# lammps/lammps-plugins

Measured on AMD Instinct MI355X. Metric: Matom-steps/sec, higher is better.
Workload: dtype f64; 1 GPU; REBO-MoS bulk: in.rebomos-bulk cell replicated 24x24x24; atoms=3981312, style=rebomos, parallelism=spatial-dd1, transport=none (one GPU), rccl_library_is_test_double=False, thermo_every=10, displacement_check=every step, deferred on-device flag, dangerous_builds=0, inner_skin=adaptive from 1.0, late_style_list_builds_rank0=0, row_prunings_late_rank0=0, rccl_ranks=1

## Files before the change

### include/mdpair_hip.h

```cpp
#ifndef MDPAIR_HIP_H
#define MDPAIR_HIP_H

#include <stddef.h>
#include <stdint.h>

#ifdef __cplusplus
extern "C" {
#endif

#define MDP_ABI_VERSION 3

enum {
  MDP_OK = 0,
  MDP_EINVAL = -1,
  MDP_EHIP = -2,
  MDP_ENOMEM = -3,
  MDP_EOVERFLOW = -4,
  MDP_ENOTIMPL = -5,
  MDP_ESTATE = -6
};

#define MDP_EFLAG_GLOBAL 1
#define MDP_EFLAG_ATOM 2
#define MDP_VFLAG_GLOBAL 1
// ... 86 lines not shown

int mdp_md_setup(mdp_ctx *ctx, const mdp_md_config *cfg, const double *x, const double *v, const int *type,
                 const int *tag, const double *mass, const int *map, const int *ghost_owner,
                 const double *ghost_shift, const int *ghost_type, const int *ghost_tag);
int mdp_md_build_neighbors(mdp_ctx *ctx);
int mdp_md_initial_integrate(mdp_ctx *ctx);
int mdp_md_final_integrate(mdp_ctx *ctx);
int mdp_md_final_initial_integrate(mdp_ctx *ctx);
int mdp_md_defer_final(mdp_ctx *ctx);
int mdp_md_compute(mdp_ctx *ctx, int eflag, int vflag);
int mdp_md_compute_begin(mdp_ctx *ctx, int eflag, int vflag);
int mdp_md_compute_end(mdp_ctx *ctx, int eflag, int vflag);
int mdp_md_pack_x(mdp_ctx *ctx, int n, const int *d_sendlist, const double *d_shift, double *d_buf);
int mdp_md_unpack_x(mdp_ctx *ctx, int first_ghost, int n, const double *d_buf);
int mdp_md_pack_scalar(mdp_ctx *ctx, int which, int n, const int *d_sendlist, double *d_buf);
int mdp_md_unpack_scalar(mdp_ctx *ctx, int which, int first_ghost, int n, const double *d_buf);
int mdp_md_pack_ghost_f(mdp_ctx *ctx, int first_ghost, int n, double *d_buf);
int mdp_md_unpack_add_f(mdp_ctx *ctx, int n, const int *d_sendlist, const double *d_buf);
int mdp_md_fold_self_ghost_f(mdp_ctx *ctx);
int mdp_md_aeam_density(mdp_ctx *ctx, int eflag);
int mdp_md_aeam_force_begin(mdp_ctx *ctx, int eflag, int vflag);
int mdp_md_aeam_force(mdp_ctx *ctx, int eflag, int vflag);
int mdp_md_aeam_state(mdp_ctx *ctx, int out[4]);
int mdp_md_thermo(mdp_ctx *ctx, double out[9]);
int mdp_md_download(mdp_ctx *ctx, double *x, double *v, double *f, double *eatom);
int mdp_md_upload_x(mdp_ctx *ctx, const double *x);
int mdp_md_download_x_all(mdp_ctx *ctx, double *x_all);
void *mdp_md_ptr(mdp_ctx *ctx, const char *name);
int mdp_md_neighbor_stats(mdp_ctx *ctx, long long out[8]);
int mdp_md_prune_stats(mdp_ctx *ctx, long long out[4]);
int mdp_md_list_state(mdp_ctx *ctx, double out[8]);
int mdp_rebomos_list_info(mdp_ctx *ctx, long long out[8]);
int mdp_rebomos_centre_paths(mdp_ctx *ctx, long long out[2], int reset);
int mdp_md_class_stats(mdp_ctx *ctx, long long out[32]);

typedef struct {
  double boxlo[3];
  double h[6];
  int procgrid[3];
  int rank;
  double cutghost;
  int self_remote;
  int nonperiodic[3];
} mdp_dd_config;

int mdp_dd_setup(mdp_ctx *ctx, const mdp_dd_config *cfg);
int mdp_dd_reneighbor(mdp_ctx *ctx);
int mdp_dd_migrate_begin(mdp_ctx *ctx, int *send_counts );
int mdp_dd_migrate_pack(mdp_ctx *ctx, double *d_buf);
int mdp_dd_migrate_end(mdp_ctx *ctx, int narrive, const double *d_buf);
int mdp_dd_borders_begin(mdp_ctx *ctx, int *send_counts );
int mdp_dd_borders_pack(mdp_ctx *ctx, double *d_buf);
int mdp_dd_borders_end(mdp_ctx *ctx, const int *recv_counts , const double *d_buf);
int mdp_dd_info(mdp_ctx *ctx, long long out[8], int *send_counts, int *recv_counts);
int mdp_dd_forward_pack(mdp_ctx *ctx, double *d_buf);
int mdp_dd_forward_unpack(mdp_ctx *ctx, const double *d_buf);
int mdp_dd_forward_scalar_pack(mdp_ctx *ctx, double *d_buf);
int mdp_dd_forward_scalar_unpack(mdp_ctx *ctx, const double *d_buf);
int mdp_dd_reverse_pack(mdp_ctx *ctx, double *d_buf);
int mdp_dd_reverse_unpack(mdp_ctx *ctx, const double *d_buf);
int mdp_dd_comm_unique_id(void *id128);
int mdp_dd_comm_library(char *buf, int cap);
int mdp_dd_comm_init(mdp_ctx *ctx, const void *id128);
int mdp_dd_comm_destroy(mdp_ctx *ctx);
int mdp_dd_comm_reneighbor(mdp_ctx *ctx);
int mdp_dd_comm_forward_begin(mdp_ctx *ctx);
// ... 175 lines not shown
```

### lammps-plugins_amd/csrc/md.hip

```cpp
#include "mdp_common.h"

#include <rocprim/rocprim.hpp>

#include <cmath>
#include <type_traits>

void mdp_rebomos_fill_dev(mdp_ctx *c, double skin);

namespace {

struct CutTables {
  double owned[MDP_AEAM_MAXT * MDP_AEAM_MAXT];
  double ghost[MDP_AEAM_MAXT * MDP_AEAM_MAXT];
  const double *g_owned;
  int ne;
  int min_type;
};

using Grid = MdpGrid;

__device__ __forceinline__ int cell_index(const Grid &g, const double4 &x, int &cx, int &cy, int &cz)
{
  cx = (int) ((x.x - g.lo[0]) * g.inv[0]);
  cy = (int) ((x.y - g.lo[1]) * g.inv[1]);
// ... 1613 lines not shown
  if (!strcmp(name, "fp")) return c->fp.p;
  if (!strcmp(name, "eatom")) return c->eatom.p;
  return nullptr;
}

int mdp_rebomos_list_info(mdp_ctx *c, long long out[8])
{
  if (!c || !out) return MDP_EINVAL;
  if (!c->rebo_packed) return mdp_fail(c, MDP_ESTATE, "rebomos lists not built yet");
  out[0] = c->lj_tiled ? 1 : 0;
  out[1] = c->ntile;
  out[2] = c->tile_cap;
  out[3] = c->tile_maxu;
  out[4] = c->lj_total;
  out[5] = c->nclus;
  out[6] = (c->lj_class_base[2] - c->lj_class_base[1]) + (c->lj_class_base[4] - c->lj_class_base[3]);
  out[7] = c->style_builds;
  return MDP_OK;
}

int mdp_rebomos_centre_paths(mdp_ctx *c, long long out[2], int reset)
{
  if (!c || !out) return MDP_EINVAL;
  out[0] = out[1] = 0;
  if (!c->centre_paths.p) return MDP_OK;
  unsigned long long h[2];
  MDP_TRY(mdp_read_one(c, c->centre_paths.p, sizeof h, h));
  out[0] = (long long) h[0];
  out[1] = (long long) h[1];
  if (reset) MDP_HIP(c, hipMemsetAsync(c->centre_paths.p, 0, sizeof h, c->stream));
  return MDP_OK;
}

int mdp_md_class_stats(mdp_ctx *c, long long out[32])
{
  if (!c || !out) return MDP_EINVAL;
  for (int k = 0; k < 32; k++) out[k] = 0;
  out[30] = c->tile_maxu;
  if (c->cfg.style == 2 || (c->have_aeam && !c->have_rebomos)) {
    out[0] = c->h_ang_count;
    out[1] = c->ntile;
    out[2] = c->aeam_split;
    return MDP_OK;
  }
  for (int k = 0; k < MDP_NCLASS; k++) out[k] = c->h_class_count[k];
  for (int k = 0; k < 4; k++) out[20 + k] = c->lj_class_base[k + 1] - c->lj_class_base[k];
  if (c->lj_tiled && !c->lj_ordered) out[20] = c->ntile;
  if (c->h_pinned) {
    const int *h = mdp_pin(c, kPinOvf) + 4 * c->ovf_par;
    for (int k = 0; k < 4; k++) out[25 + k] = h[k];
    out[24] = *mdp_pin(c, kPinGeneral);
  }
  out[29] = c->tile_small;
  return MDP_OK;
}

int mdp_md_neighbor_stats(mdp_ctx *c, long long out[8])
{
  if (!c || !out) return MDP_EINVAL;
  for (int k = 0; k < 8; k++) out[k] = 0;
  out[0] = c->nb_owned_total;
  out[1] = c->nb_total - c->nb_owned_total;
  out[2] = c->lj_total;
  out[3] = c->cand_total;
  out[4] = 0;
  for (int k = 0; k < MDP_NCLASS; k++) out[4] += c->h_class_count[k];
// ... 110 lines not shown
```

### lammps-plugins_amd/csrc/rebomos.hip

```cpp
#include "mdp_common.h"

#include <type_traits>

#define MDP_SINPI_COEFFS 3.14159265358979312e+00, -5.16771278004996937e+00, 2.55016403987734508e+00, -5.99264529320791883e-01, 8.21458866111281910e-02, -7.37043094571434784e-03, 4.66302805767612337e-04, -2.19153534478302037e-05
#define MDP_COSPI_COEFFS 1.00000000000000000e+00, -4.93480220054467900e+00, 4.05871212641676760e+00, -1.33526276885458928e+00, 2.35330630358893123e-01, -2.58068913900140508e-02, 1.92957430940392206e-03, -1.04638104924845650e-04, 4.30306958703294391e-06
__constant__ double mdp_sinpi_series[8] = {MDP_SINPI_COEFFS};
__constant__ double mdp_cospi_series[9] = {MDP_COSPI_COEFFS};

namespace {

#ifndef MDP_LJ_WAVES
#define MDP_LJ_WAVES 4
#endif
constexpr double kPi = 3.14159265358979323846;
constexpr double kTol = 1.0e-9;

__device__ __forceinline__ void wave_lds_fence()
{
  __builtin_amdgcn_fence(__ATOMIC_RELEASE, "wavefront");
  __builtin_amdgcn_wave_barrier();
  __builtin_amdgcn_fence(__ATOMIC_ACQUIRE, "wavefront");
}

template <int G> __device__ __forceinline__ double group_sum_any(double v, const int s, const int lane);
// ... 362 lines not shown
    q[5] = dw;
    q[REC == kRec ? 8 : kInvF] = rinv;
    je[pos] = t | (tj << 30);
    nsum += w;
  }
  n += __popcll(gb);
  if (base < 64) active |= gb << base;
}

__device__ __forceinline__ double bpermute_f64(const int addr4, const double v)
{
  const int lo = __builtin_amdgcn_ds_bpermute(addr4, __double2loint(v));
  const int hi = __builtin_amdgcn_ds_bpermute(addr4, __double2hiint(v));
  return __hiloint2double(hi, lo);
}

template <int K> __device__ __forceinline__ double unread_f64()
{
  double v;
  asm("; unread value %1" : "=v"(v) : "n"(K));
  return v;
}

template <int G> struct CentreCfg {
  static constexpr int CAP = G;
  static constexpr int GPW = 64 / G;
  static constexpr int WPB = G == 12 ? 3 : 4;
  static constexpr int STRIDE = CAP * kRecF + 2;
  static constexpr int MSTRIDE = 2 * (G / 2) * G + 2;
  static constexpr int UA = G >= 32 ? 1 : (G >= 12 ? 2 : 4);
};


template <int G, bool LIST = false>
__global__ __launch_bounds__(64 * CentreCfg<G>::WPB) void rebo_centre_kernel(
    const RebomosDev P, const int *__restrict__ centres, const int ncent_arg, const int nlocal,
    const double4 *__restrict__ xq, const int *__restrict__ cand_off, const int *__restrict__ cand,
    const int *__restrict__ pk, unsigned long long *__restrict__ amask, double *__restrict__ fnbr,
    double *__restrict__ fown, double *__restrict__ acc, int *__restrict__ ovf, const int eflag, const int vflag,
    const int tc ,
    const int full_on ,
    unsigned long long *__restrict__ path_cnt )
{
  using C = CentreCfg<G>;
  __shared__ double s_rec[C::WPB * C::GPW * C::STRIDE];
  __shared__ double s_mat[C::WPB * C::GPW * C::MSTRIDE];
  __shared__ int s_je[C::WPB * C::GPW * C::CAP];

  const int tid = threadIdx.x;
  const int lane = tid & 63;
  const int s = lane % G;
  const int glane0 = lane - s;
  const int gw = lane / G;
  const bool lane_ok = gw < C::GPW;
  const int grp_in_block = (tid >> 6) * C::GPW + (lane_ok ? gw : C::GPW - 1);
  const long long gid = (long long) (LIST ? (int) blockIdx.x : xcd_contiguous(blockIdx.x, gridDim.x)) * (C::WPB * C::GPW) + grp_in_block;
  const int ncent = LIST ? centres[-1] : ncent_arg;
  const bool have = lane_ok && gid < ncent;
  if (LIST) {
    int *h_count = reinterpret_cast<int *>(const_cast<int *>(pk));
    if (blockIdx.x == 0 && tid == 0) *h_count = ncent;
    const long long covered = (long long) gridDim.x * (C::WPB * C::GPW);
    for (long long e = covered + (long long) blockIdx.x * blockDim.x + tid; e < ncent; e += (long long) gridDim.x * blockDim.x)
      ovf[1 + atomicAdd(&ovf[0], 1)] = centres[e];
  }

  double *rec = s_rec + (size_t) grp_in_block * C::STRIDE;
// ... 84 lines not shown
  int tcc = tc;
  asm volatile("; centre constants from here" : "+s"(tcc));
#pragma unroll
  for (int k = 0; k < 7; k++) {
    cb[k] = P.b[tcc][k];
    cg[k] = P.bg[tcc][k];
  }
  const double ea = exp(-P.a[tcc][2] * Ntot);
  const double dp = -P.a[tcc][0] + P.a[tcc][1] * P.a[tcc][2] * ea;
  const double PS = -P.a[tcc][0] * (Ntot - 1.0) - P.a[tcc][1] * ea + P.a[tcc][3];

  const SeriesLead lead = series_lead();
  const int nw = wave_max_int(n);
  CentreOut o = {0, 0, 0, 0, 0, 0, 0};

  const double ux = mx * mri, uy = my * mri, uz = mz * mri;
  const int lane_base = (threadIdx.x & 63) - s;
  constexpr bool kFullPath = G <= 16;
  constexpr bool kAllLanes = C::GPW * G == 64;
  const int lane_again = (int) __builtin_amdgcn_mbcnt_hi(~0u, __builtin_amdgcn_mbcnt_lo(~0u, 0u));
  bool full = false;
  if constexpr (kFullPath) full = full_on && __all(!lane_ok || n == G);
  if (path_cnt && __any(have) && lane == 0) atomicAdd(&path_cnt[full ? 0 : 1], 1ull);
  const double *qm = rec + m * kRecF;
  const double *qwrap = qm - G * kRecF;
  double *em = mat + 2 * m;
  int from4[kFullPath ? G / 2 : 1];
  if constexpr (kFullPath)
    if (full) {
#pragma unroll
      for (int d = 1; d <= G / 2; d++) from4[d - 1] = 4 * (lane - d + (m < d ? G : 0));
    }
  double S = 0.0;
  if (full) {
    if constexpr (kFullPath)
      if (kAllLanes || lane_again < C::GPW * G) {
#pragma unroll
        for (int d = 1; d <= G / 2; d++) {
          const bool half = 2 * d == G;
          const double *q = (m >= G - d ? qwrap : qm) + d * kRecF;
          double give = unread_f64<0>();
          if (!half || m < d) {
            double cs = (ux * q[0] + uy * q[1] + uz * q[2]) * q[kInvF];
            cs = fmin(cs, 1.0);
            cs = fmax(cs, -1.0);
            double dg, g;
            if (__any(cs >= 0.5)) g = gspline(cb, cg, cs, dg, lead);
            else g = poly6(cb, cs, dg);
            em[2 * (d - 1) * G] = g;
            em[2 * (d - 1) * G + 1] = dg;
            S += q[4] * g;
            give = mw * g;
          }
          const double got = bpermute_f64(from4[d - 1], give);
          if (!half || m >= d) S += got;
          __builtin_amdgcn_sched_barrier(0);
        }
      }
  } else
  for (int d = 1; d <= nw / 2; d++) {
    const bool mine = act && (2 * d < n || (2 * d == n && m < d));
    double give = 0.0;
    if (mine) {
      int qi = m + d;
      qi = qi >= n ? qi - n : qi;
      const double *q = rec + qi * kRecF;
      double cs = (ux * q[0] + uy * q[1] + uz * q[2]) * q[kInvF];
      cs = fmin(cs, 1.0);
      cs = fmax(cs, -1.0);
      double dg, g;
      if (__any(cs >= 0.5)) g = gspline(cb, cg, cs, dg, lead);
      else g = poly6(cb, cs, dg);
      double *e = mat + 2 * ((d - 1) * G + m);
      e[0] = g;
      e[1] = dg;
      S += q[4] * g;
      give = mw * g;
    }
    int src = m - d;
    src = src < 0 ? src + n : src;
    const double got = __shfl(give, lane_base + (act ? src : m), 64);
    S += act ? got : 0.0;
  }
  double mC = 0.0, mp = 0.0, mVA = 0.0;
  if (act) {
    const PairPar pp = pair_par(P, tc);
    const int tm = ((unsigned) je[m]) >> 30;
    mp = rsqrt_nr(1.0 + S + PS);
    mVA = -mw * pp.B(tm) * exp(-pp.beta(tm) * mr);
    mC = (mw > kTol) ? 0.5 * mVA * (-0.5 * mp * mp * mp) : 0.0;
    rec[m * kRecF + 6] = mC;
// ... 1663 lines not shown
  const long long i64 = (long long) blockIdx.x * (256 / RP_L) + threadIdx.x / RP_L + (MODE == 1 ? nlocal : 0);
  bool have = i64 < (MODE == 0 ? nlocal : nall);
  const int i = have ? (int) i64 : 0;
  if (MODE == 1 && have && !is_centre[i]) have = false;
  const double4 xi = xq[i];
  const int ti = (int) xi.w;
  if (ti < 0) have = false;
  const long long b = have ? nb_off[i] : 0;
  const int len = have ? (int) (nb_off[i + 1] - b) : 0;
  const int lenw = wave_max_int(len);
  int *stage = have ? stage_all + (size_t) i * kCandStride : nullptr;
  const unsigned long long below = (1ull << s) - 1ull;
  int n = 0;
  for (int base = 0; base < lenw; base += RP_L) {
    const int k = base + s;
    bool keep = false;
    int j = 0;
    if (k < len) {
      j = nb[b + k];
      const double4 xj = xq[j];
      const double dx = xi.x - xj.x, dy = xi.y - xj.y, dz = xi.z - xj.z;
      const int tj = (int) xj.w;
      keep = j != i && tj >= 0 && (dx * dx + dy * dy + dz * dz) <= P.cand_cutsq[ti * 2 + tj];
    }
    const unsigned long long bk = (__ballot(keep) >> glane0) & 0xFFFFull;
    if (keep) {
      const int pos = n + __popcll(bk & below);
      if (pos < kCandStride) stage[pos] = j;
      if (MODE == 0 && j >= mark_from) is_centre[j] = 1;
    }
    n += __popcll(bk);
  }
  if (have && s == 0) cnt[i] = n;
}

__global__ __launch_bounds__(256) void rev_kernel(const int nlocal, const int *__restrict__ cand_off,
                                                  const int *__restrict__ cand, int *__restrict__ rev,
                                                  int *__restrict__ rev16, int *__restrict__ flags,
                                                  const int self_end, const double4 *__restrict__ xq,
                                                  const int *__restrict__ tag, const int *__restrict__ ghost_owner,
                                                  const RebomosDev P)
{
  const int s = threadIdx.x % RP_L;
  const long long a64 = (long long) blockIdx.x * (256 / RP_L) + threadIdx.x / RP_L;
  if (a64 >= nlocal) return;
  const int a = (int) a64;
  const int off = cand_off[a], nc = cand_off[a + 1] - off;
  if (nc > 64 && s == 0) atomicOr(&flags[1], 1);
  for (int t = s; t < nc; t += RP_L) {
    const int j = cand[off + t];
    int r = -1;
    if (j >= nlocal && j < self_end) {
      const int o = ghost_owner[j - nlocal];
      const double4 xa = xq[a], xj = xq[j], xo = xq[o];
      const double px = xa.x - (xj.x - xo.x), py = xa.y - (xj.y - xo.y), pz = xa.z - (xj.z - xo.z);
      const int ta = tag[a];
      const int oo = cand_off[o], no = cand_off[o + 1] - oo;
      for (int u = 0; u < no; u++) {
        const int k = cand[oo + u];
        if (tag[k] != ta) continue;
        const double4 xk = xq[k];
        const double ex = xk.x - px, ey = xk.y - py, ez = xk.z - pz;
        if (ex * ex + ey * ey + ez * ez < 1.0e-6) {
          r = oo + u;
          break;
        }
// ... 346 lines not shown
    MDP_TRY(mdp_launch(c, count, nblk(nclus, 16), 256, 0, c->stream, c->grid, c->rebomos, nclus, c->nlocal, c->xq.p,
                       c->cell_perm.p, c->cell_start.p, c->lj_cnt.p, c->lj_split.p, nullptr, nullptr));
  MDP_TRY(mdp_scan_exclusive_i64(c, c->lj_cnt.p, c->lj_off.p, nclus));
  const MdpRead rd[2] = {cand_read, {c->lj_off.p + nclus, sizeof(long long), &c->lj_total}};
  MDP_TRY(mdp_read_small(c, rd, 2));
  MDP_HIP(c, c->lj.reserve((size_t) c->lj_total + 1));
  if (nclus)
    MDP_TRY(mdp_launch(c, fill, nblk(nclus, 16), 256, 0, c->stream, c->grid, c->rebomos, nclus, c->nlocal, c->xq.p,
                       c->cell_perm.p, c->cell_start.p, c->lj_cnt.p, c->lj_split.p, c->lj_off.p, c->lj.p));
  mdp_rows_renewed(c);
  return MDP_OK;
}

static int repack_cand_fill(mdp_ctx *c, const Repack &R)
{
  const int nall = c->nall, nlocal = c->nlocal, cand_total = R.cand_total;
  hipStream_t st = c->stream;
  c->cand_total = cand_total;
  MDP_HIP(c, c->cand.reserve((size_t) cand_total + 1));
  MDP_HIP(c, c->rev.reserve((size_t) cand_total + 1));
  MDP_HIP(c, c->rev16.reserve((size_t) 16 * nlocal + 16));
  MDP_HIP(c, c->fnbr.reserve((size_t) 4 * cand_total + 4));
  MDP_HIP(c, c->fown.reserve((size_t) 4 * nall + 4));
  MDP_HIP(c, hipMemsetAsync(c->fown.p, 0, sizeof(double) * 4 * nall, st));
  if (nall && R.stage)
    MDP_TRY(mdp_launch(c, cand_compact_kernel, nblk(nall, kRpPerBlock), 256, 0, st, nall, c->cand_off.p, R.stage, c->cand.p));
  else if (nall)
    MDP_TRY(mdp_launch(c, cand_build_kernel<2>, nblk(nall, kRpPerBlock), 256, 0, st, c->grid, R.Rc, c->rebomos, nall, nlocal,
                       c->xq.p, c->cell_perm.p, c->cell_start.p, nullptr, c->cand_off.p, c->cand.p, c->is_center.p, R.self_end,
                       c->xq_cell.p));
  return MDP_OK;
}

static int repack_launch_classes(mdp_ctx *c)
{
  hipStream_t st = c->stream;
  const bool tiled = c->lj_tiled;
  const int nunit = tiled ? c->ntile : c->nclus;
  c->lj_ordered = false;
  for (int q = 0; q <= 4; q++) c->lj_class_base[q] = q ? nunit : 0;
  int kSmallUnion = 1210;
  if (const char *e = getenv("MDP_TILE_SMALL")) kSmallUnion = atoi(e) > 0 ? atoi(e) : kSmallUnion;
  c->tile_small = tiled ? (c->tile_maxu < kSmallUnion ? c->tile_maxu : kSmallUnion) : 0;
  if (!(nunit > 0 && tiled && c->tile_maxu > kSmallUnion)) return MDP_OK;
  MDP_HIP(c, c->cl_flag.reserve((size_t) 6 * (nunit + 1)));
  MDP_HIP(c, c->cl_pos.reserve((size_t) 4 * (nunit + 2)));
  MDP_HIP(c, c->cl_order.reserve(nunit + 1));
  int *flag4 = c->cl_flag.p;
  MDP_TRY(mdp_launch(c, unit_class_kernel, nblk(nunit), 256, 0, st, nunit, nullptr, c->tile_nu.p, kSmallUnion, flag4));
  int total[4] = {0, 0, 0, 0};
  MdpRead rd[4];
  for (int q = 0; q < 4; q++) {
    int *pos = c->cl_pos.p + (size_t) q * (nunit + 2);
    MDP_TRY(mdp_scan_exclusive_int(c, flag4 + (size_t) q * (nunit + 1), pos, nunit));
    rd[q] = {pos + nunit, sizeof(int), &total[q]};
  }
  MDP_TRY(mdp_read_small(c, rd, 4));
  for (int q = 0; q < 4; q++) c->lj_class_base[q + 1] = c->lj_class_base[q] + total[q];
  MDP_TRY(mdp_launch(c, unit_order_kernel, nblk(nunit), 256, 0, st, nunit, flag4, c->cl_pos.p, c->lj_class_base[1],
                     c->lj_class_base[2], c->lj_class_base[3], c->cl_order.p));
  c->lj_ordered = true;
  return MDP_OK;
}

static int repack_centres(mdp_ctx *c, const Repack &R, bool *overflow)
{
// ... 39 lines not shown
    for (int g = 0; g < MDP_NCLASS_HALF; g++) {
      const int n0 = c->h_class_count[g], n1 = c->h_class_count[g + MDP_NCLASS_HALF];
      if (n0)
        MDP_HIP(c, hipMemcpyAsync(c->class_merged.p + c->merged_base[g], c->class_list.p + (size_t) g * nall, sizeof(int) * n0,
                                  hipMemcpyDeviceToDevice, st));
      if (n1)
        MDP_HIP(c, hipMemcpyAsync(c->class_merged.p + c->merged_base[g] + n0,
                                  c->class_list.p + (size_t) (g + MDP_NCLASS_HALF) * nall, sizeof(int) * n1,
                                  hipMemcpyDeviceToDevice, st));
    }
  }
  for (int k = 0; k < MDP_NCLASS; k++) {
    const int w = width[(k % MDP_NCLASS_HALF) / 2];
    const long long n = (long long) c->h_class_count[k] * w;
    if (n > 0)
      MDP_TRY(mdp_launch(c, pack_cand_kernel, nblk(n), 256, 0, st, c->h_class_count[k], w, c->class_list.p + (size_t) k * nall,
                         c->cand_off.p, c->cand.p, c->pk_cand.p + c->pk_base[k]));
  }
  return MDP_OK;
}

int mdp_rebomos_repack(mdp_ctx *c)
{
  if (!c->have_rebomos) return mdp_fail(c, MDP_ESTATE, "rebomos parameters not set");
  if (!c->atoms_set) return mdp_fail(c, MDP_ESTATE, "atoms not set");
  c->host_check_armed = false;
  Repack R;
  bool overflow = false;
  repack_inner_skin(c);
  MDP_TRY(repack_setup(c, R));
  MDP_TRY(repack_cand_count(c, R));
  MDP_TRY(repack_lj_rows(c, R));
  MDP_TRY(repack_cand_fill(c, R));
  MDP_TRY(repack_launch_classes(c));
  MDP_TRY(repack_centres(c, R, &overflow));
  if (overflow) {
    if (getenv("MDP_DIAG")) repack_diag(c);
    if (c->skin_inner > 0.2 + 1e-9 && !getenv("MDP_INNER_SKIN")) {
      fprintf(stderr, "[mdp] rebomos: a candidate row (atoms within rcmax + inner skin) outgrew 64 entries at an inner skin "
                      "of %.2f A; the style's lists are rebuilt with %.2f A and keep that cap (mdp_md_list_state)\n",
              c->skin_inner, 0.5 * c->skin_inner > 0.2 ? 0.5 * c->skin_inner : 0.2);
      c->skin_inner_cap = c->skin_inner;
      c->skin_inner_auto = 0.5 * c->skin_inner > 0.2 ? 0.5 * c->skin_inner : 0.2;
      c->stale_rebuild = false;
      return mdp_rebomos_repack(c);
    }
    return mdp_fail(c, MDP_EOVERFLOW, "rebomos: an atom has more than 64 neighbours inside rcmax+skin (Neighbor list overflow)");
  }
  c->rebo_packed = true;
  c->style_builds++;
  return MDP_OK;
}


static int rebomos_check_launch(mdp_ctx *c, const double trig)
{
  const int nall = c->nall;
  const double hard = 0.5 * c->skin_inner;
  int *h = mdp_pin(c, kPinHostCheck);
  h[0] = h[1] = h[2] = h[3] = 0;
  const bool pr = c->prune_valid;
  double ptrig = 0.5 * c->prune_buf - kPruneMargin * mdp_margin_scale(c);
  if (ptrig < 0.25 * c->prune_buf) ptrig = 0.25 * c->prune_buf;
  const double phard = 0.5 * c->prune_buf;
  return mdp_moved(c, nall, 2048, trig * trig, hard * hard, c->xhold_all.p, h, pr ? c->xhold_prune.p : nullptr,
                   ptrig * ptrig, phard * phard);
// ... 13 lines not shown
  stale = false;
  if (!c->nall) return MDP_OK;
  int *h = mdp_pin(c, kPinHostCheck);
  if (!c->md && c->host_check_armed) {
    c->host_check_armed = false;
    stale = h[0] != 0;
    if (c->prune_valid && h[2]) c->prune_stale = true;
    return MDP_OK;
  }
  const bool deferred_host = !c->md && c->hn_on && c->hn_deferred_check && !c->check_now;
  if ((!c->md && !deferred_host) || c->check_now) {
    mdp_sflag_drop(c);
    c->check_now = false;
    MDP_TRY(rebomos_check_launch(c, 0.5 * c->skin_inner));
    MDP_HIP(c, hipStreamSynchronize(c->stream));
    stale = h[0] != 0;
    if (c->prune_valid && h[2]) c->prune_stale = true;
    return MDP_OK;
  }
  bool toofar = false;
  MDP_TRY(mdp_sflag_collect(c, &stale, &toofar));
  if (toofar) c->dangerous_builds++;
  return MDP_OK;
}

static int centre_path_mode(mdp_ctx *c)
{
  const char *fe = getenv("MDP_CENTRE_FULL");
  c->centre_full_now = !(fe && atoi(fe) == 0);
  const char *ce = getenv("MDP_CENTRE_COUNT");
  c->centre_cnt_now = nullptr;
  if (ce && atoi(ce) != 0) {
    if (!c->centre_paths.p) {
      MDP_HIP(c, c->centre_paths.reserve(2));
      MDP_HIP(c, hipMemsetAsync(c->centre_paths.p, 0, sizeof(unsigned long long) * 2, c->stream));
    }
    c->centre_cnt_now = c->centre_paths.p;
  }
  return MDP_OK;
}

template <int G>
static void launch_centre(mdp_ctx *c, int kg, int eflag, int vflag, int part)
{
  for (int elem = 0; elem < 2; elem++) {
    const int k = 2 * kg + elem + (part == 1 ? MDP_NCLASS_HALF : 0);
    const int n = c->h_class_count[k] + (part == 2 ? c->h_class_count[k + MDP_NCLASS_HALF] : 0);
    if (n <= 0) continue;
    const int *list = part == 2 ? c->class_merged.p + c->merged_base[k] : c->class_list.p + (size_t) k * c->nall;
    constexpr int per_block = CentreCfg<G>::WPB * CentreCfg<G>::GPW;
    const int grid = (n + per_block - 1) / per_block;
    rebo_centre_kernel<G><<<grid, 64 * CentreCfg<G>::WPB, 0, c->stream>>>(c->rebomos, list, n, c->nlocal,
                                                       c->xq.p, c->cand_off.p, c->cand.p, c->pk_cand.p + c->pk_base[k],
                                                       c->amask.p, c->fnbr.p, c->fown.p, c->acc.p, c->ovf.p, eflag, vflag,
                                                       elem, c->centre_full_now ? 1 : 0, c->centre_cnt_now);
  }
}

static void launch_centre3(mdp_ctx *c, int eflag, int vflag, int part)
{
  for (int elem = 0; elem < 2; elem++) {
    const int k = elem + (part == 1 ? MDP_NCLASS_HALF : 0);
    const int n = c->h_class_count[k] + (part == 2 ? c->h_class_count[k + MDP_NCLASS_HALF] : 0);
    if (n <= 0) continue;
    const int *clist = part == 2 ? c->class_merged.p + c->merged_base[k] : c->class_list.p + (size_t) k * c->nall;
    const int q = (part == 1 ? 2 : 0) + elem;
    int *list = c->ovf.p + (size_t) (q + 1) * c->ovf_stride + 1;
    int *h_cnt = mdp_pin(c, kPinOvf) + 4 * c->ovf_par + q;
    if (*h_cnt > 0) c->ovf3_hot[q] = 64;
    else if (c->ovf3_hot[q] > 0) c->ovf3_hot[q]--;
    const bool list_mode = c->ovf3_hot[q] > 0;
    rebo_centre3_kernel<<<(n + kC3Block - 1) / kC3Block, kC3Block, 0, c->stream>>>(c->rebomos, clist, n,
                                                                c->nlocal, c->xq.p, c->cand_off.p, c->cand.p,
                                                                c->pk_cand.p + c->pk_base[k], c->amask.p, c->fnbr.p,
                                                                c->fown.p, c->acc.p, list, list_mode ? nullptr : c->ovf.p,
                                                                eflag, vflag, elem);
    if (!list_mode) continue;
    constexpr int per_block = CentreCfg<8>::WPB * CentreCfg<8>::GPW;
    long long est = 4 * (long long) *h_cnt + 2 * per_block;
    if (est > n) est = n;
    const int grid = (int) ((est + per_block - 1) / per_block);
    rebo_centre_kernel<8, true><<<grid, 64 * CentreCfg<8>::WPB, 0, c->stream>>>(
        c->rebomos, list, 0, c->nlocal, c->xq.p, c->cand_off.p, c->cand.p, h_cnt, c->amask.p, c->fnbr.p, c->fown.p,
        c->acc.p, c->ovf.p, eflag, vflag, elem, c->centre_full_now ? 1 : 0, c->centre_cnt_now);
  }
}

static bool lj_queue_mode(mdp_ctx *c)
{
  const char *fe = getenv("MDP_LJ_QUEUE");
  const int forced = fe ? (atoi(fe) != 0 ? 1 : 0) : -1;
  bool on = false;
  if (c->lj_tiled && c->cluster == 2 && c->ntile > 0 && forced != 0) {
    const int listed = *mdp_pin(c, kPinCubic);
    on = forced == 1 || (long long) listed * 8 > c->ntile;
  }
  const char *ce0 = getenv("MDP_LJ_QUEUE_CAP");
  const bool recap = ce0 && c->lj_cq_cap && atoi(ce0) >= 1 && atoi(ce0) <= 4096 && atoi(ce0) != c->lj_cq_cap;
  if (on && (c->lj_cq_tiles != c->ntile || !c->lj_cq.p || recap)) {
    int kCap = 64;
    if (const char *ce = getenv("MDP_LJ_QUEUE_CAP")) kCap = atoi(ce) >= 1 && atoi(ce) <= 4096 ? atoi(ce) : kCap;
    if (c->lj_cq.reserve((size_t) c->ntile * MDP_TILE * 2 * kCap + 8) != hipSuccess ||
        c->lj_cq_cnt.reserve((size_t) c->ntile * MDP_TILE * 2 + 8) != hipSuccess ||
        hipMemsetAsync(c->lj_cq_cnt.p, 0, sizeof(int) * ((size_t) c->ntile * MDP_TILE * 2 + 8), c->stream) != hipSuccess)
      on = false;
    else {
      c->lj_cq_cap = kCap;
      c->lj_cq_tiles = c->ntile;
    }
  }
  c->lj_queue_now = on;
  return on;
}

static int launch_lj(mdp_ctx *c, int klass, bool gather, int eflag, int vflag, bool accumulate)
// ... 210 lines not shown
```

### lammps-plugins_amd/host/capi.py

```python
from __future__ import annotations

import ctypes as C
import os

import numpy as np

PKG_DIR = os.path.dirname(os.path.dirname(os.path.abspath(__file__)))
LIB_PATH = os.path.join(PKG_DIR, "libmdpair_hip.so")

D22 = (C.c_double * 2) * 2


class RebomosParams(C.Structure):
    _fields_ = [(n, D22) for n in ("rcmin", "rcmax", "rcmaxsq", "Q", "alpha", "A", "BIJc", "Beta")] + [
        ("b", (C.c_double * 2) * 7), ("bg", (C.c_double * 2) * 7), ("a", (C.c_double * 2) * 4)] + [
        (n, D22) for n in ("rcLJmin", "rcLJmax", "epsilon", "sigma", "lj1", "lj2", "lj3", "lj4")]


class AeamTables(C.Structure):
    _fields_ = [("ntypes", C.c_int), ("nelements", C.c_int), ("nnonangular", C.c_int),
                ("nrhomax", C.c_int), ("nrmax", C.c_int), ("nfrho", C.c_int), ("nrhor", C.c_int), ("nz2r", C.c_int),
                ("nrho", C.POINTER(C.c_int)), ("drho", C.POINTER(C.c_double)),
                ("nr", C.POINTER(C.c_int)), ("dr", C.POINTER(C.c_double)), ("cut", C.POINTER(C.c_double)),
                ("type2frho", C.POINTER(C.c_int)), ("type2rhor", C.POINTER(C.c_int)), ("type2z2r", C.POINTER(C.c_int)),
# ... 62 lines not shown

EXPORTS = [
    "mdp_abi_version", "mdp_device_count", "mdp_create", "mdp_destroy", "mdp_last_error", "mdp_set_stream",
    "mdp_sync", "mdp_rebomos_set_params", "mdp_rebomos_read_file", "mdp_rebomos_params_from_scalars",
    "mdp_aeam_set_tables", "mdp_aeam_file_read", "mdp_aeam_file_info", "mdp_aeam_file_build", "mdp_aeam_file_free", "mdp_set_atoms_host", "mdp_set_positions_host",
    "mdp_set_box_host", "mdp_host_ghosts_derived",
    "mdp_set_neighbors_host", "mdp_set_skin", "mdp_set_neighbors_csr_host", "mdp_rebomos_compute_host", "mdp_aeam_density_host",
    "mdp_aeam_force_host", "mdp_md_setup", "mdp_md_build_neighbors", "mdp_md_initial_integrate",
    "mdp_md_final_integrate", "mdp_md_final_initial_integrate", "mdp_md_compute", "mdp_md_compute_begin", "mdp_md_compute_end", "mdp_md_pack_x", "mdp_md_unpack_x", "mdp_md_pack_scalar",
    "mdp_md_unpack_scalar", "mdp_md_pack_ghost_f", "mdp_md_unpack_add_f", "mdp_md_fold_self_ghost_f",
    "mdp_md_aeam_density", "mdp_md_aeam_force", "mdp_md_thermo", "mdp_md_download", "mdp_md_upload_x", "mdp_md_ptr",
    "mdp_md_neighbor_stats", "mdp_md_class_stats", "mdp_md_prune_stats", "mdp_hnve_setup", "mdp_hnve_off", "mdp_hnve_upload_v",
    "mdp_hnve_initial", "mdp_hnve_final", "mdp_hnve_download", "mdp_rebomos_list_info", "mdp_set_timing", "mdp_get_timing",
    "mdp_device_bytes", "mdp_host_release", "mdp_rebomos_check_host_list",
    "mdp_dd_setup", "mdp_dd_reneighbor", "mdp_dd_migrate_begin", "mdp_dd_migrate_pack", "mdp_dd_migrate_end",
    "mdp_dd_borders_begin", "mdp_dd_borders_pack", "mdp_dd_borders_end", "mdp_dd_info", "mdp_dd_forward_pack",
    "mdp_dd_forward_unpack", "mdp_dd_forward_scalar_pack", "mdp_dd_forward_scalar_unpack", "mdp_dd_reverse_pack",
    "mdp_dd_reverse_unpack", "mdp_md_moved_async", "mdp_md_integrate_check", "mdp_md_download_int", "mdp_md_download_x_all",
    "mdp_dd_comm_unique_id", "mdp_dd_comm_library", "mdp_dd_comm_init", "mdp_dd_comm_destroy", "mdp_dd_comm_reneighbor",
    "mdp_dd_comm_forward_begin", "mdp_dd_comm_forward_end", "mdp_dd_comm_forward_scalar", "mdp_dd_comm_reverse",
    "mdp_dd_comm_allreduce", "mdp_dd_comm_step_begin", "mdp_dd_comm_step_end", "mdp_dd_comm_step_info", "mdp_aeam_device_lists", "mdp_rebomos_host_list", "mdp_aeam_check_host_list",
    "mdp_md_defer_final", "mdp_md_list_state", "mdp_md_aeam_force_begin", "mdp_md_aeam_state", "mdp_dd_comm_aeam_exchange_begin", "mdp_dd_comm_aeam_exchange_end",
    "mdp_nhc_setup", "mdp_nhc_run", "mdp_nhc_state", "mdp_nhc_set_state", "mdp_nhc_off",
    "mdp_langevin_setup", "mdp_langevin_run", "mdp_langevin_tally", "mdp_langevin_off",
    "mdp_langevin_baths", "mdp_langevin_tally_bath",
    "mdp_fire_setup", "mdp_fire_iterate", "mdp_fire_state", "mdp_fire_off",
    "mdp_md_set_mask", "mdp_hnve_set_mask", "mdp_integrate_group", "mdp_langevin_group",
    "mdp_md_set_image", "mdp_md_download_unwrapped", "mdp_msd_setup", "mdp_msd_sums", "mdp_msd_info", "mdp_msd_off",
    "mdp_rdf_setup", "mdp_rdf_counts", "mdp_rdf_info", "mdp_rdf_off",
    "mdp_adf_setup", "mdp_adf_counts", "mdp_adf_info", "mdp_adf_off",
    "mdp_coord_setup", "mdp_coord_read", "mdp_coord_info", "mdp_coord_off",
    "mdp_centro_setup", "mdp_centro_read", "mdp_centro_info", "mdp_centro_off",
    "mdp_profile_setup", "mdp_profile_range", "mdp_profile_exponent", "mdp_profile_sums", "mdp_profile_info", "mdp_profile_off",
    "mdp_rebomos_centre_paths",
    "mdp_heatflux_sums", "mdp_md_download_vatom",
    "mdp_heat_setup", "mdp_heat_run", "mdp_heat_state", "mdp_heat_off",
    "mdp_indent_setup", "mdp_indent_run", "mdp_indent_state", "mdp_indent_off",
    "mdp_spring_setup", "mdp_spring_run", "mdp_spring_state", "mdp_spring_off",
]


class MdpError(RuntimeError):
    def __init__(self, code, text):
        super().__init__(f"libmdpair_hip: error {code}: {text}")
        self.code = code


_lib = None


def lib():
    global _lib
    if _lib is None:
        if not os.path.exists(LIB_PATH):
            raise FileNotFoundError(f"{LIB_PATH} not built: run `python __graft_entry__.py` (make -C lammps-plugins_amd)")
        try:
            import torch
        except ImportError:
            pass
        _lib = C.CDLL(os.environ.get("MDP_LIB_PATH") or LIB_PATH)
        _lib.mdp_last_error.restype = C.c_char_p
        _lib.mdp_md_ptr.restype = C.c_void_p
        _lib.mdp_device_bytes.restype = C.c_double
    return _lib


def profile_exponent(rng, natoms_total):
# ... 299 lines not shown
    def md_download(self, nlocal, want=("x", "v", "f")):
        arrs = {k: (np.zeros((nlocal, 3)) if k in want else None) for k in ("x", "v", "f")}
        ea = np.zeros(nlocal) if "eatom" in want else None
        self._ck(self.L.mdp_md_download(self.h, _dp(arrs["x"]), _dp(arrs["v"]), _dp(arrs["f"]), _dp(ea)))
        arrs["eatom"] = ea
        return arrs

    def md_download_x_all(self, nall):
        x = np.zeros((max(nall, 1), 3))
        self._ck(self.L.mdp_md_download_x_all(self.h, _dp(x)))
        return x[:nall]

    def md_upload_x(self, x):
        x = np.ascontiguousarray(x, dtype=np.float64)
        self._ck(self.L.mdp_md_upload_x(self.h, _dp(x)))

    def md_ptr(self, name: str) -> int:
        p = self.L.mdp_md_ptr(self.h, name.encode())
        if not p:
            raise MdpError(-1, f"mdp_md_ptr({name}) returned NULL")
        return int(p)

    def rebomos_list_info(self):
        out = (C.c_longlong * 8)()
        self._ck(self.L.mdp_rebomos_list_info(self.h, out))
        keys = ("tiled", "tiles", "union_stride", "union_max", "row_entries", "clusters", "large_tiles", "builds")
        return dict(zip(keys, (int(v) for v in out)))

    def rebomos_centre_paths(self, reset=True):
        out = (C.c_longlong * 2)()
        self._ck(self.L.mdp_rebomos_centre_paths(self.h, out, C.c_int(1 if reset else 0)))
        return int(out[0]), int(out[1])

    def md_neighbor_stats(self):
        out = (C.c_longlong * 8)()
        self._ck(self.L.mdp_md_neighbor_stats(self.h, out))
        return list(out)

    def hnve_setup(self, dt, ftm2v, mass_per_type):
        m = np.ascontiguousarray(mass_per_type, dtype=np.float64)
        self._ck(self.L.mdp_hnve_setup(self.h, C.c_double(dt), C.c_double(ftm2v), _dp(m), C.c_int(len(m) - 1)))

    def hnve_off(self):
        self._ck(self.L.mdp_hnve_off(self.h))

    def hnve_upload_v(self, v):
        v = np.ascontiguousarray(v, dtype=np.float64)
        self._ck(self.L.mdp_hnve_upload_v(self.h, _dp(v)))

    def hnve_initial(self):
        m, d = C.c_int(0), C.c_int(0)
        self._ck(self.L.mdp_hnve_initial(self.h, C.byref(m), C.byref(d)))
        return bool(m.value), bool(d.value)

    def hnve_final(self):
        self._ck(self.L.mdp_hnve_final(self.h))

    def hnve_download(self, nlocal, want=("x", "v", "f")):
        out = {k: np.zeros((nlocal, 3)) for k in want}
        self._ck(self.L.mdp_hnve_download(self.h, _dp(out.get("x")), _dp(out.get("v")), _dp(out.get("f"))))
        return out

    def nhc_setup(self, t_start, t_stop, t_period, nf, tchain=3, tloop=1, drag=0.0, boltz=BOLTZ_METAL, mvv2e=1.0364269e-4):
        cfg = NhcConfig(t_start, t_stop, t_period, tchain, tloop, drag, nf, boltz, mvv2e)
        self._ck(self.L.mdp_nhc_setup(self.h, C.byref(cfg)))

# ... 503 lines not shown
```

Measured before the change: 1522 Matom-steps/s.

## Order REBO candidate lists by azimuth to cut divergent spline branches

Adds a kernel that runs after each candidate-list fill. It sorts every atom's candidate neighbours by azimuth around the axis of least spread, with height as the tie-breaker. The goal is that, in the full-path centre kernel, the lane pairs with a fixed offset rarely reach cos>=0.5, so whole waves can take the cheap poly6 branch instead of gspline. It also adds an optional counter of blend trips plus a profiling script. The cost is an O(n^2) rank sort with atan2 at every rebuild, and the changed neighbour order may change memory locality and floating-point summation order.

```diff
diff --git a/include/mdpair_hip.h b/include/mdpair_hip.h
--- a/include/mdpair_hip.h
+++ b/include/mdpair_hip.h
@@ -142,6 +142,7 @@
 int mdp_md_list_state(mdp_ctx *ctx, double out[8]);
 int mdp_rebomos_list_info(mdp_ctx *ctx, long long out[8]);
 int mdp_rebomos_centre_paths(mdp_ctx *ctx, long long out[2], int reset);
+int mdp_rebomos_centre_blend_trips(mdp_ctx *ctx, long long *out, int reset);
 int mdp_md_class_stats(mdp_ctx *ctx, long long out[32]);
 
 typedef struct {
diff --git a/lammps-plugins_amd/csrc/md.hip b/lammps-plugins_amd/csrc/md.hip
--- a/lammps-plugins_amd/csrc/md.hip
+++ b/lammps-plugins_amd/csrc/md.hip
@@ -1669,6 +1669,18 @@
   return MDP_OK;
 }
 
+int mdp_rebomos_centre_blend_trips(mdp_ctx *c, long long *out, int reset)
+{
+  if (!c || !out) return MDP_EINVAL;
+  *out = 0;
+  if (!c->centre_paths.p) return MDP_OK;
+  unsigned long long h;
+  MDP_TRY(mdp_read_one(c, c->centre_paths.p + 2, sizeof h, &h));
+  *out = (long long) h;
+  if (reset) MDP_HIP(c, hipMemsetAsync(c->centre_paths.p + 2, 0, sizeof h, c->stream));
+  return MDP_OK;
+}
+
 int mdp_md_class_stats(mdp_ctx *c, long long out[32])
 {
   if (!c || !out) return MDP_EINVAL;
diff --git a/lammps-plugins_amd/csrc/rebomos.hip b/lammps-plugins_amd/csrc/rebomos.hip
--- a/lammps-plugins_amd/csrc/rebomos.hip
+++ b/lammps-plugins_amd/csrc/rebomos.hip
@@ -418,7 +418,7 @@
 };
 
 
-template <int G, bool LIST = false>
+template <int G, bool LIST = false, bool COUNT = false>
 __global__ __launch_bounds__(64 * CentreCfg<G>::WPB) void rebo_centre_kernel(
     const RebomosDev P, const int *__restrict__ centres, const int ncent_arg, const int nlocal,
     const double4 *__restrict__ xq, const int *__restrict__ cand_off, const int *__restrict__ cand,
@@ -569,6 +569,7 @@
       for (int d = 1; d <= G / 2; d++) from4[d - 1] = 4 * (lane - d + (m < d ? G : 0));
     }
   double S = 0.0;
+  int blend = 0;
   if (full) {
     if constexpr (kFullPath)
       if (kAllLanes || lane_again < C::GPW * G) {
@@ -582,8 +583,10 @@
             cs = fmin(cs, 1.0);
             cs = fmax(cs, -1.0);
             double dg, g;
-            if (__any(cs >= 0.5)) g = gspline(cb, cg, cs, dg, lead);
-            else g = poly6(cb, cs, dg);
+            if (__any(cs >= 0.5)) {
+              g = gspline(cb, cg, cs, dg, lead);
+              if constexpr (COUNT) blend++;
+            } else g = poly6(cb, cs, dg);
             em[2 * (d - 1) * G] = g;
             em[2 * (d - 1) * G + 1] = dg;
             S += q[4] * g;
@@ -594,6 +597,8 @@
           __builtin_amdgcn_sched_barrier(0);
         }
       }
+    if constexpr (COUNT)
+      if (path_cnt && blend && lane == 0) atomicAdd(&path_cnt[2], (unsigned long long) blend);
   } else
   for (int d = 1; d <= nw / 2; d++) {
     const bool mine = act && (2 * d < n || (2 * d == n && m < d));
@@ -2323,6 +2328,76 @@
     n += __popcll(bk);
   }
   if (have && s == 0) cnt[i] = n;
+}
+
+constexpr int kOrderRow = 64;
+__global__ __launch_bounds__(256) void cand_order_kernel(const RebomosDev P, const int nall,
+                                                         const double4 *__restrict__ xq,
+                                                         const int *__restrict__ cand_off, int *__restrict__ cand)
+{
+  constexpr int NG = 256 / RP_L, U = kOrderRow / RP_L;
+  __shared__ double s_az[NG][kOrderRow], s_h[NG][kOrderRow];
+  const int s = threadIdx.x % RP_L, grp = threadIdx.x / RP_L;
+  const long long i64 = (long long) blockIdx.x * NG + grp;
+  int off = 0, nc = 0;
+  if (i64 < nall) {
+    off = cand_off[i64];
+    nc = cand_off[i64 + 1] - off;
+  }
+  if (nc > kOrderRow) nc = 0;
+  const double4 xi = xq[nc ? (int) i64 : 0];
+  const int ti = (int) xi.w;
+  double dx[U], dy[U], dz[U], sxx = 0.0, syy = 0.0, szz = 0.0;
+  int jj[U];
+#pragma unroll
+  for (int u = 0; u < U; u++) {
+    const int t = u * RP_L + s;
+    jj[u] = -1;
+    dx[u] = dy[u] = dz[u] = 0.0;
+    if (t < nc) {
+      jj[u] = cand[off + t];
+      const double4 xj = xq[jj[u]];
+      dx[u] = xj.x - xi.x;
+      dy[u] = xj.y - xi.y;
+      dz[u] = xj.z - xi.z;
+      if (dx[u] * dx[u] + dy[u] * dy[u] + dz[u] * dz[u] < P.rcmaxsq[ti * 2 + (int) xj.w]) {
+        sxx += dx[u] * dx[u];
+        syy += dy[u] * dy[u];
+        szz += dz[u] * dz[u];
+      }
+    }
+  }
+#pragma unroll
+  for (int o = RP_L / 2; o > 0; o >>= 1) {
+    sxx += __shfl_xor(sxx, o, 64);
+    syy += __shfl_xor(syy, o, 64);
+    szz += __shfl_xor(szz, o, 64);
+  }
+  const int axis = (szz <= sxx && szz <= syy) ? 2 : (syy <= sxx ? 1 : 0);
+#pragma unroll
+  for (int u = 0; u < U; u++) {
+    const int t = u * RP_L + s;
+    if (t < nc) {
+      const double a = axis == 2 ? dx[u] : (axis == 1 ? dz[u] : dy[u]);
+      const double b = axis == 2 ? dy[u] : (axis == 1 ? dx[u] : dz[u]);
+      s_az[grp][t] = atan2(b, a);
+      s_h[grp][t] = axis == 2 ? dz[u] : (axis == 1 ? dy[u] : dx[u]);
+    }
+  }
+  __syncthreads();
+#pragma unroll
+  for (int u = 0; u < U; u++) {
+    const int t = u * RP_L + s;
+    if (t < nc) {
+      const double az = s_az[grp][t], h = s_h[grp][t];
+      int rank = 0;
+      for (int k = 0; k < nc; k++) {
+        const double ak = s_az[grp][k], hk = s_h[grp][k];
+        rank += (ak < az || (ak == az && (hk < h || (hk == h && k < t)))) ? 1 : 0;
+      }
+      cand[off + rank] = jj[u];
+    }
+  }
 }
 
 __global__ __launch_bounds__(256) void rev_kernel(const int nlocal, const int *__restrict__ cand_off,
@@ -2735,6 +2810,14 @@
   return MDP_OK;
 }
 
+static int repack_cand_order(mdp_ctx *c)
+{
+  const char *e = getenv("MDP_CAND_ORDER");
+  if ((e && atoi(e) == 0) || !c->nall || !c->cand_total) return MDP_OK;
+  return mdp_launch(c, cand_order_kernel, nblk(c->nall, kRpPerBlock), 256, 0, c->stream, c->rebomos, c->nall, c->xq.p,
+                    c->cand_off.p, c->cand.p);
+}
+
 static int repack_launch_classes(mdp_ctx *c)
 {
   hipStream_t st = c->stream;
@@ -2840,6 +2923,7 @@
   MDP_TRY(repack_cand_count(c, R));
   MDP_TRY(repack_lj_rows(c, R));
   MDP_TRY(repack_cand_fill(c, R));
+  MDP_TRY(repack_cand_order(c));
   MDP_TRY(repack_launch_classes(c));
   MDP_TRY(repack_centres(c, R, &overflow));
   if (overflow) {
@@ -2919,8 +3003,8 @@
   c->centre_cnt_now = nullptr;
   if (ce && atoi(ce) != 0) {
     if (!c->centre_paths.p) {
-      MDP_HIP(c, c->centre_paths.reserve(2));
-      MDP_HIP(c, hipMemsetAsync(c->centre_paths.p, 0, sizeof(unsigned long long) * 2, c->stream));
+      MDP_HIP(c, c->centre_paths.reserve(3));
+      MDP_HIP(c, hipMemsetAsync(c->centre_paths.p, 0, sizeof(unsigned long long) * 3, c->stream));
     }
     c->centre_cnt_now = c->centre_paths.p;
   }
@@ -2937,10 +3021,11 @@
     const int *list = part == 2 ? c->class_merged.p + c->merged_base[k] : c->class_list.p + (size_t) k * c->nall;
     constexpr int per_block = CentreCfg<G>::WPB * CentreCfg<G>::GPW;
     const int grid = (n + per_block - 1) / per_block;
-    rebo_centre_kernel<G><<<grid, 64 * CentreCfg<G>::WPB, 0, c->stream>>>(c->rebomos, list, n, c->nlocal,
-                                                       c->xq.p, c->cand_off.p, c->cand.p, c->pk_cand.p + c->pk_base[k],
-                                                       c->amask.p, c->fnbr.p, c->fown.p, c->acc.p, c->ovf.p, eflag, vflag,
-                                                       elem, c->centre_full_now ? 1 : 0, c->centre_cnt_now);
+    const auto kernel = c->centre_cnt_now ? rebo_centre_kernel<G, false, true> : rebo_centre_kernel<G>;
+    kernel<<<grid, 64 * CentreCfg<G>::WPB, 0, c->stream>>>(c->rebomos, list, n, c->nlocal, c->xq.p, c->cand_off.p, c->cand.p,
+                                                           c->pk_cand.p + c->pk_base[k], c->amask.p, c->fnbr.p, c->fown.p,
+                                                           c->acc.p, c->ovf.p, eflag, vflag, elem,
+                                                           c->centre_full_now ? 1 : 0, c->centre_cnt_now);
   }
 }
 
@@ -2967,7 +3052,8 @@
     long long est = 4 * (long long) *h_cnt + 2 * per_block;
     if (est > n) est = n;
     const int grid = (int) ((est + per_block - 1) / per_block);
-    rebo_centre_kernel<8, true><<<grid, 64 * CentreCfg<8>::WPB, 0, c->stream>>>(
+    const auto kernel8 = c->centre_cnt_now ? rebo_centre_kernel<8, true, true> : rebo_centre_kernel<8, true>;
+    kernel8<<<grid, 64 * CentreCfg<8>::WPB, 0, c->stream>>>(
         c->rebomos, list, 0, c->nlocal, c->xq.p, c->cand_off.p, c->cand.p, h_cnt, c->amask.p, c->fnbr.p, c->fown.p,
         c->acc.p, c->ovf.p, eflag, vflag, elem, c->centre_full_now ? 1 : 0, c->centre_cnt_now);
   }
diff --git a/lammps-plugins_amd/host/capi.py b/lammps-plugins_amd/host/capi.py
--- a/lammps-plugins_amd/host/capi.py
+++ b/lammps-plugins_amd/host/capi.py
@@ -118,7 +118,7 @@
     "mdp_coord_setup", "mdp_coord_read", "mdp_coord_info", "mdp_coord_off",
     "mdp_centro_setup", "mdp_centro_read", "mdp_centro_info", "mdp_centro_off",
     "mdp_profile_setup", "mdp_profile_range", "mdp_profile_exponent", "mdp_profile_sums", "mdp_profile_info", "mdp_profile_off",
-    "mdp_rebomos_centre_paths",
+    "mdp_rebomos_centre_paths", "mdp_rebomos_centre_blend_trips",
     "mdp_heatflux_sums", "mdp_md_download_vatom",
     "mdp_heat_setup", "mdp_heat_run", "mdp_heat_state", "mdp_heat_off",
     "mdp_indent_setup", "mdp_indent_run", "mdp_indent_state", "mdp_indent_off",
@@ -484,6 +484,11 @@
         self._ck(self.L.mdp_rebomos_centre_paths(self.h, out, C.c_int(1 if reset else 0)))
         return int(out[0]), int(out[1])
 
+    def rebomos_centre_blend_trips(self, reset=True):
+        out = C.c_longlong(0)
+        self._ck(self.L.mdp_rebomos_centre_blend_trips(self.h, C.byref(out), C.c_int(1 if reset else 0)))
+        return int(out.value)
+
     def md_neighbor_stats(self):
         out = (C.c_longlong * 8)()
         self._ck(self.L.mdp_md_neighbor_stats(self.h, out))
diff --git a/profiles/slot_order/trip_sets.py b/profiles/slot_order/trip_sets.py
--- /dev/null
+++ b/profiles/slot_order/trip_sets.py
@@ -0,0 +1,68 @@
+import os
+import sys
+from collections import Counter
+
+import numpy as np
+
+ROOT = os.path.dirname(os.path.dirname(os.path.dirname(os.path.abspath(__file__))))
+sys.path.insert(0, ROOT)
+import __graft_entry__ as entry
+
+entry.load_package()
+from lammps_plugins_amd.host import capi, system as S
+
+
+def neighbours(s, rc):
+    xa, type_all, _, _, _, _, _ = S.with_ghosts(s, float(np.max(rc)) + 0.5)
+    rc2 = rc[0][type_all - 1] ** 2
+    out = []
+    for i in np.flatnonzero(s.type == 1):
+        d = xa - xa[i]
+        r2 = (d ** 2).sum(axis=1)
+        out.append(d[(r2 < rc2) & (r2 > 0.0)])
+    return out
+
+
+def azimuth_order(d):
+    sxx, syy, szz = (d ** 2).sum(axis=0)
+    axis = 2 if (szz <= sxx and szz <= syy) else (1 if syy <= sxx else 0)
+    a, b = {2: (0, 1), 1: (2, 0), 0: (1, 2)}[axis]
+    az = np.arctan2(d[:, b], d[:, a])
+    return np.lexsort((np.arange(len(d)), d[:, axis], az))
+
+
+def sweep_order(d):
+    return np.lexsort((d[:, 0], d[:, 1], d[:, 2]))
+
+
+def trips(d):
+    n = len(d)
+    u = d / np.linalg.norm(d, axis=1)[:, None]
+    cs = u @ u.T
+    hit = set()
+    for k in range(1, n // 2 + 1):
+        ms = range(n) if 2 * k < n else range(k)
+        if any(cs[m, (m + k) % n] >= 0.5 for m in ms):
+            hit.add(k)
+    return tuple(sorted(hit))
+
+
+def main():
+    p = capi.read_rebomos_file(os.path.join(ROOT, "tests", "golden", "potentials", "MoS.REBO.set5b"))
+    rc = np.array([[p.rcmax[a][b] for b in range(2)] for a in range(2)])
+    base = S.replicate(S.rebomos_bulk_cell(), (4, 4, 2))
+    rng = np.random.default_rng(8)
+    for name, s in (("lattice", base),
+                    ("Gaussian jitter 0.08 A", S.System(base.box, S.wrap(base.box, base.x + rng.normal(0.0, 0.08, base.x.shape)),
+                                                         base.type, base.tag, base.mass))):
+        nb = neighbours(s, rc)
+        for oname, order in (("sweep order", sweep_order), ("azimuth order", azimuth_order)):
+            sets = Counter()
+            for d in nb:
+                if len(d) == 12:
+                    sets[trips(d[order(d)])] += 1
+            print(f"{name}, {oname}: " + ", ".join(f"{n} centres {set(k) if k else '{}'}" for k, n in sorted(sets.items())))
+
+
+if __name__ == "__main__":
+    main()
```

New measurement: 1569 Matom-steps/s (median of 6 runs). +3.1%, better.
